# whwu95/MVFNet

Measured on AMD Instinct MI355X. Metric: clips/sec (fwd+bwd) MVFNet-R50 8x8 224^2, higher is better.
Workload: dtype bf16; 1 GPU; MVFNet-ResNet50 8x8, 32 clips/GPU of 8x3x224x224, bf16, train step: fwd (batch-stat BN) + loss + bwd + clip + SGD-nesterov; all through the HIP C ABI (stem + 16 bottlenecks + MVF + TSN head); clips_per_gpu=32, frames_per_clip=8, parallelism=dp1: replicas, one flat gradient all-reduce per step

## Files before the change

### mvfnet_amd/csrc/conv_nhwc.hip

```cpp
#include <algorithm>
#include <type_traits>
#include <stdlib.h>
#include <string.h>

#include "common.h"

namespace {

constexpr int kThreads = 256;
constexpr int kPitch = 144;
constexpr int kBM = 128;

typedef float f32x16 __attribute__((ext_vector_type(16)));
typedef short bf16x8 __attribute__((ext_vector_type(8)));

struct ConvArgs {
    const char* x;
    const char* x2;
    const char* w;
    const char* res;
    const float* bias;
    char* y;
    int N, H, W, Cin, Cout, KH, KW, stride, pad, Ho, Wo;
    int xps, split_c, x2ps, relu;
// ... 742 lines not shown
            }
        }
        if (wm == 0) __builtin_amdgcn_s_barrier();
        asm volatile("s_waitcnt vmcnt(0)" ::: "memory");
        __syncthreads();
#undef MVF_PIN2
    } else if constexpr (GLDS >= 2) {
        if (nseg > 0) load_chunk(s0, 0);
        for (int kc = 0; kc < nseg; ++kc) {
            asm volatile("s_waitcnt vmcnt(0)" ::: "memory");
            __syncthreads();
#ifdef MVF_CONV_ABLATE
            if (kc + 1 < nseg && !(a.prio & 4)) load_chunk(s0, (kc + 1) & 1);
            if (!(a.prio & 2)) compute(kc & 1);
#else
            if constexpr (ILV) {
                const bool more = kc + 1 < nseg;
                if (more) prep_chunk((kc + 1) & 1);
                compute(kc & 1, more);
            } else {
                if (kc + 1 < nseg) load_chunk(s0, (kc + 1) & 1);
                compute(kc & 1);
            }
#endif
        }
        __syncthreads();
    } else if constexpr (LOWK) {
        if (nseg > 0) {
            load_chunk(s0);
            store_chunk(0, s0);
        }
        __syncthreads();
        for (int kc = 0; kc < nseg; ++kc) {
            const bool more = kc + 1 < nseg;
            if (more) load_chunk(s0);
            compute(0);
            if (more) {
                __syncthreads();
                store_chunk(0, s0);
            }
            __syncthreads();
        }
    } else if constexpr (PF2) {
        load_chunk(s0);
        load_chunk(s1);
        if (nseg > 0) store_chunk(0, s0);
        __syncthreads();
        load_chunk(s0);
        int kc = 0;
        for (; kc + 1 < nseg; kc += 2) {
            compute(0);
            store_chunk(1, s1);
            load_chunk(s1);
            __syncthreads();
            compute(1);
            if (kc + 2 < nseg) store_chunk(0, s0);
            load_chunk(s0);
            __syncthreads();
        }
        if (kc < nseg) {
            compute(0);
            __syncthreads();
        }
    } else {
        if (nseg > 0) {
            load_chunk(s0);
            store_chunk(0, s0);
        }
        __syncthreads();
        for (int kc = 0; kc < nseg; ++kc) {
            const int buf = kc & 1;
            const bool more = kc + 1 < nseg;
            if (more) load_chunk(s0);
            compute(buf);
            if (more) store_chunk(buf ^ 1, s0);
            __syncthreads();
        }
    }

#ifdef MVF_CONV_ABLATE
    if (a.prio & 16) return;
#endif
    if (mode == SEG_PRODUCE) {
        float* slot = sk.ws + (long)g_self * (BM * BN);
#pragma unroll
        for (int i = 0; i < TM; ++i)
#pragma unroll
            for (int j = 0; j < TN; ++j)
#pragma unroll
                for (int r = 0; r < 16; ++r) slot[((i * TN + j) * 16 + r) * NT + tid] = acc[i][j][r];
        asm volatile("s_waitcnt vmcnt(0)" ::: "memory");
        __syncthreads();
        if (tid == 0) {
            __builtin_amdgcn_fence(__ATOMIC_RELEASE, "agent");
            asm volatile("s_waitcnt vmcnt(0)" ::: "memory");
            __hip_atomic_store(sk.flags + g_self, 1u, __ATOMIC_RELAXED, __HIP_MEMORY_SCOPE_AGENT);
        }
        return;
    }
    if (mode == SEG_FINISH) {
        for (int g = g_first; g < g_self; ++g) {
            if (tid == 0) {
                unsigned spins = 0;
                while (__hip_atomic_load(sk.flags + g, __ATOMIC_RELAXED, __HIP_MEMORY_SCOPE_AGENT) == 0u) {
                    __builtin_amdgcn_s_sleep(4);
                    if (++spins > (1u << 26)) {
                        __hip_atomic_store(sk.err, 1u, __ATOMIC_RELAXED, __HIP_MEMORY_SCOPE_AGENT);
                        break;
                    }
                }
                __builtin_amdgcn_fence(__ATOMIC_ACQUIRE, "agent");
            }
            __syncthreads();
            const float* slot = sk.ws + (long)g * (BM * BN);
#pragma unroll
            for (int i = 0; i < TM; ++i)
#pragma unroll
                for (int j = 0; j < TN; ++j)
#pragma unroll
                    for (int r = 0; r < 16; ++r) acc[i][j][r] += slot[((i * TN + j) * 16 + r) * NT + tid];
        }
    }

    const bool e_bias = EPI == 0 ? a.bias != nullptr : (EPI == 4 || EPI == 5 || (EPI == 6 && a.bias != nullptr));
    const bool e_res = EPI == 0 ? a.res != nullptr : (EPI == 3 || EPI == 5 || EPI == 8 || EPI == 9 || EPI == 10 || EPI == 12);
    constexpr bool e_bw = EPI == 9 || EPI == 10;
    const bool e_relu = EPI == 0 ? a.relu != 0 : (EPI == 4 || EPI == 5);
    constexpr bool e_apply = EPI == 8;
    const bool e_stats = EPI == 0 ? a.stats_part != nullptr : (EPI == 1 || EPI == 12);
    constexpr bool e_bnb = EPI == 6;
    const bool e_scatter = (EPI == 0 || EPI == 6) && a.o_s > 0;
    constexpr int CP = BN * 4 + 16;
    constexpr int NH = (LOWK || GLDS) ? 2 : 1;
    constexpr int HR = BM / NH;
    static_assert(HR * CP <= kSmem, "C tile (or half) must fit in the A/B LDS buffers");
    static_assert(HR % 32 == 0, "half split follows the MFMA row tiles");
    constexpr int PPT = BM / kBM;
    constexpr int HPP = NH / PPT;
    static_assert(NH % PPT == 0 && HPP >= 1, "a statistics partial covers whole epilogue passes");
    constexpr int TPR = BN / 4, RPP = NT / TPR;
    const int cq = tid % TPR, r0 = tid / TPR;
    const int col = n0 + cq * 4;
    ET* y = reinterpret_cast<ET*>(a.y);
    const ET* res = reinterpret_cast<const ET*>(a.res);
    float4 bv = make_float4(0.f, 0.f, 0.f, 0.f);
    if (e_bias && col < a.Cout) bv = *reinterpret_cast<const float4*>(a.bias + col);
    float4 st1 = make_float4(0.f, 0.f, 0.f, 0.f), st2 = st1, kk = st1;
    if (e_stats && a.stats_shift && col < a.Cout) kk = *reinterpret_cast<const float4*>(a.stats_shift + col);
    float4 ap_s = st1, ap_b = st1, ap_rs = make_float4(1.f, 1.f, 1.f, 1.f), ap_rb = st1;
    if (e_apply && col < a.Cout) {
        ap_s = *reinterpret_cast<const float4*>(a.ap_scale + col); ap_b = *reinterpret_cast<const float4*>(a.ap_shift + col);
        if (a.ap_rscale) { ap_rs = *reinterpret_cast<const float4*>(a.ap_rscale + col); ap_rb = *reinterpret_cast<const float4*>(a.ap_rshift + col); }
    }
    float4 b_mu = st1, b_rs = st1, b_sc = st1, b_sh = st1;
    if (e_bnb && col < a.Cout) {
        b_mu = *reinterpret_cast<const float4*>(a.bn_mean + col); b_rs = *reinterpret_cast<const float4*>(a.bn_invstd + col);
        b_sc = *reinterpret_cast<const float4*>(a.bn_scale + col); b_sh = *reinterpret_cast<const float4*>(a.bn_shift + col);
    }
    float4 w_a = st1, w_d0 = st1, w_kx = st1;
    if (e_bw && col < a.Cout) {
        b_mu = *reinterpret_cast<const float4*>(a.bn_mean + col); b_rs = *reinterpret_cast<const float4*>(a.bn_invstd + col);
        if constexpr (EPI == 9) {
            const float inv_m = 1.0f / (float)a.M;
            const float4 ga = *reinterpret_cast<const float4*>(a.bw_gamma + col), dg = *reinterpret_cast<const float4*>(a.bw_dgamma + col),
                         db = *reinterpret_cast<const float4*>(a.bw_dbeta + col);
            w_a = make_float4(ga.x * b_rs.x, ga.y * b_rs.y, ga.z * b_rs.z, ga.w * b_rs.w);
            w_d0 = make_float4(db.x * inv_m, db.y * inv_m, db.z * inv_m, db.w * inv_m);
            w_kx = make_float4(b_rs.x * dg.x * inv_m, b_rs.y * dg.y * inv_m, b_rs.z * dg.z * inv_m, b_rs.w * dg.w * inv_m);
        }
    }
    typedef unsigned u32x2 __attribute__((ext_vector_type(2)));
    const int eimg0 = fd_div(m0, a.fd_hw_mul, a.fd_hw_shr);
    __amdgpu_buffer_rsrc_t rs_y, rs_res;
    {
        const long total = (e_scatter ? (long)a.N * a.o_hfull * a.o_wfull : (long)a.M) * a.Cout * ESZ;
        const long base = (e_scatter ? (long)eimg0 * a.o_hfull * a.o_wfull : (long)m0) * a.Cout * ESZ;
        const long left = total - base;
        const unsigned nrec = (unsigned)(left < 0x7ffffff0L ? left : 0x7ffffff0L);
        rs_y = __builtin_amdgcn_make_buffer_rsrc((void*)(a.y + base), 0, a.y ? nrec : 0u, 0x00020000);
        rs_res = __builtin_amdgcn_make_buffer_rsrc((void*)(e_res ? a.res + base : (e_bnb ? a.bn_z + base : a.y + base)), 0, nrec, 0x00020000);
    }
    const __amdgpu_buffer_rsrc_t rs_mask = __builtin_amdgcn_make_buffer_rsrc(
        (void*)(a.res_mask ? a.res_mask + (long)m0 * (a.Cout / 4) : (const unsigned char*)a.y), 0,
        (unsigned)min((long)(a.M - m0) * (a.Cout / 4), 0x7ffffff0L), 0x00020000);
    const __amdgpu_buffer_rsrc_t rs_gate = __builtin_amdgcn_make_buffer_rsrc(
        (void*)(a.out_gate ? a.out_gate + (long)m0 * (a.Cout / 4) : (const unsigned char*)a.y), 0,
        (unsigned)min((long)(a.M - m0) * (a.Cout / 4), 0x7ffffff0L), 0x00020000);
    const bool e_gate = e_res && !e_apply && !e_bw && a.out_gate != nullptr;
    (void)y; (void)res;
    constexpr int kMaskOff = HR * CP;
    constexpr int MSEG = BN / 64;
    static_assert(kMaskOff + BM * (BN / 4) <= kSmem, "mask tile must fit behind the C tile");
    const bool mask_lds = e_res && (a.res_mask || e_gate) && (a.Cout % 64 == 0) && a.mask_lds;
    if (mask_lds) {
#pragma unroll
        for (int it = tid; it < BM * MSEG; it += NT) {
            const int row = it / MSEG, seg = it - row * MSEG;
            const unsigned moff = (unsigned)(row * (a.Cout / 4) + n0 / 4 + seg * 16);
            u32x4 mv = {0x0f0f0f0fu, 0x0f0f0f0fu, 0x0f0f0f0fu, 0x0f0f0f0fu};
            if (a.res_mask) mv = __builtin_amdgcn_raw_buffer_load_b128(rs_mask, moff, 0, 0);
            if (e_gate) {
                const u32x4 gv = __builtin_amdgcn_raw_buffer_load_b128(rs_gate, moff, 0, 0);
                mv.x = (mv.x & 0x0f0f0f0fu) | ((gv.x & 0x0f0f0f0fu) << 4); mv.y = (mv.y & 0x0f0f0f0fu) | ((gv.y & 0x0f0f0f0fu) << 4);
// ... 503 lines not shown
        default: return false;
    }
}

template <typename ET, int WM, int WN, int TM, int TN, int EPI>
void launch_lowk(bool pw, int tiles, size_t lds, hipStream_t st, const ConvArgs& a) {
    if constexpr (sizeof(ET) == 4) {
        if (x3_on(a)) {
            constexpr size_t lds3 = (size_t)kLowkLdsX3<WM * TM * 32, WN * TN * 32>();
            if constexpr (WN * TN * 32 == 128 && EPI >= 1 && EPI <= 6) {
                const int t_wide = ((a.M + 255) / 256) * a.tiles_n;
                if (g_x3_wide > 0 && t_wide >= g_x3_wide) {
                    ConvArgs b = a;
                    b.tiles_m = (a.M + 255) / 256;
                    constexpr size_t ldsw = (size_t)kLowkLdsX3<256, 128>();
                    auto k0 = conv_igemm_x3w_kernel<EPI, false>;
                    auto k1 = conv_igemm_x3w_kernel<EPI, true>;
                    static bool attrw = false;
                    if (!attrw) {
                        (void)hipFuncSetAttribute((const void*)k0, hipFuncAttributeMaxDynamicSharedMemorySize, (int)ldsw);
                        (void)hipFuncSetAttribute((const void*)k1, hipFuncAttributeMaxDynamicSharedMemorySize, (int)ldsw);
                        attrw = true;
                    }
                    if (pw) hipLaunchKernelGGL(k1, dim3(t_wide), dim3(512), ldsw, st, b);
                    else hipLaunchKernelGGL(k0, dim3(t_wide), dim3(512), ldsw, st, b);
                    return;
                }
            }
            if constexpr (EPI >= 1 && EPI <= 6) {
                if (a.nchunks >= g_x3_db_min) {
                    constexpr size_t ldsdb = (size_t)2 * (WM * TM * 32 + WN * TN * 32) * 192;
                    auto k0 = conv_igemm_x3db_kernel<WM, WN, TM, TN, EPI, false>;
                    auto k1 = conv_igemm_x3db_kernel<WM, WN, TM, TN, EPI, true>;
                    static bool attr = false;
                    if (!attr) {
                        (void)hipFuncSetAttribute((const void*)k0, hipFuncAttributeMaxDynamicSharedMemorySize, (int)ldsdb);
                        (void)hipFuncSetAttribute((const void*)k1, hipFuncAttributeMaxDynamicSharedMemorySize, (int)ldsdb);
                        attr = true;
                    }
                    if (pw) hipLaunchKernelGGL(k1, dim3(tiles), dim3(kThreads), ldsdb, st, a);
                    else hipLaunchKernelGGL(k0, dim3(tiles), dim3(kThreads), ldsdb, st, a);
                    return;
                }
            }
            if (pw) hipLaunchKernelGGL((conv_igemm_x3_kernel<WM, WN, TM, TN, EPI, true>), dim3(tiles), dim3(kThreads), lds3, st, a);
            else hipLaunchKernelGGL((conv_igemm_x3_kernel<WM, WN, TM, TN, EPI, false>), dim3(tiles), dim3(kThreads), lds3, st, a);
            return;
        }
    }
    if (pw) {
        auto k = conv_igemm_lowk_kernel<ET, WM, WN, TM, TN, EPI, true>;
        hipLaunchKernelGGL(k, dim3(tiles), dim3(kThreads), lds, st, a);
    } else {
        auto k = conv_igemm_lowk_kernel<ET, WM, WN, TM, TN, EPI, false>;
        hipLaunchKernelGGL(k, dim3(tiles), dim3(kThreads), lds, st, a);
    }
}

template <typename ET, int WM, int WN, int TM, int TN>
__global__ __launch_bounds__(kThreads) void conv_streamk_kernel(ConvArgs a, SkArgs sk) {
    extern __shared__ __attribute__((aligned(16))) char smem[];
    const int g = blockIdx.x, nc = a.nchunks;
    auto start_of = [&](int w) { return w < sk.units_rem ? w * (sk.units_base + 1) : sk.units_rem * (sk.units_base + 1) + (w - sk.units_rem) * sk.units_base; };
    auto wg_of = [&](int u) {
        const int bnd = sk.units_rem * (sk.units_base + 1);
        return u < bnd ? u / (sk.units_base + 1) : sk.units_rem + (u - bnd) / sk.units_base;
    };
    const int u0 = start_of(g), u1 = start_of(g + 1);
    const int t_first = u0 / nc, t_last = (u1 - 1) / nc;
    const int cb_first = u0 - t_first * nc, ce_last = u1 - t_last * nc;
    const bool last_partial = ce_last < nc;
    if (last_partial) {
        const int cb = t_last == t_first ? cb_first : 0;
        conv_tile<ET, WM, WN, TM, TN>(a, smem, sk.tile0 + t_last, cb, ce_last, SEG_PRODUCE, sk, 0, g);
    }
    const int t_hi = last_partial ? t_last - 1 : t_last;
    for (int t = t_first + 1; t <= t_hi; ++t) conv_tile<ET, WM, WN, TM, TN>(a, smem, sk.tile0 + t, 0, nc, SEG_FULL, sk, 0, g);
    if (t_first <= t_hi) {
        if (cb_first == 0) conv_tile<ET, WM, WN, TM, TN>(a, smem, sk.tile0 + t_first, 0, nc, SEG_FULL, sk, 0, g);
        else conv_tile<ET, WM, WN, TM, TN>(a, smem, sk.tile0 + t_first, cb_first, nc, SEG_FINISH, sk, wg_of(t_first * nc), g);
    }
}

template <typename ET>
__global__ void pack_weight_kernel(const float* w, int cout, int cin, int kh, int kw, int kwp, int cinp,
                                   const float* scale, ET* out) {
    const long total = (long)cout * kh * kwp * cinp;
    for (long i = (long)blockIdx.x * blockDim.x + threadIdx.x; i < total; i += (long)gridDim.x * blockDim.x) {
        long t = i;
        const int ci = (int)(t % cinp); t /= cinp;
        const int x = (int)(t % kwp); t /= kwp;
        const int yk = (int)(t % kh); t /= kh;
        const int co = (int)t;
        float v = 0.f;
        if (ci < cin && x < kw) {
            v = w[(((long)co * cin + ci) * kh + yk) * kw + x];
            if (scale) v *= scale[co];
        }
        stf(out + i, v);
    }
}

__global__ void bn_fold_kernel(const float* gamma, const float* beta, const float* mean, const float* var, float eps,
                               int c, float* scale, float* shift) {
    int i = blockIdx.x * blockDim.x + threadIdx.x;
    if (i >= c) return;
    const float s = gamma[i] / sqrtf(var[i] + eps);
    scale[i] = s;
    shift[i] = beta[i] - mean[i] * s;
}

static inline bool contiguous_ok(const ConvArgs& a) { return a.o_s <= 0; }
struct SkHost {
    void* ws;
    size_t ws_bytes;
};

int g_lowk_max_chunks = 1 << 30;
int g_pf2_mode = 1;
int g_glds1_f32_infer = 1;
int g_glds1_max = -1;
int g_big_min = 0;
int g_big2_min = 16;
int g_glds_min = -1, g_glds_nb = 2;

int sk_slots() {
    static int slots = 0;
    if (!slots) {
        g_lowk_max_chunks = mvf_policy_int("conv_lowk", g_lowk_max_chunks);
        g_pf2_mode = mvf_policy_int("conv_pf2", g_pf2_mode);
        g_glds1_f32_infer = mvf_policy_int("conv_glds1_f32", g_glds1_f32_infer);
        g_glds1_max = mvf_policy_int("conv_glds1", g_glds1_max);
        g_f32_x3 = mvf_policy_int("f32_x3", g_f32_x3);
        g_x3_wide = mvf_policy_int("x3_wide", g_x3_wide);
        g_x3_db_min = mvf_policy_int("x3_db", g_x3_db_min);
        g_big_min = mvf_policy_int("conv_big", g_big_min);
        g_big2_min = mvf_policy_int("conv_big2", g_big2_min);
        g_glds_min = mvf_policy_int("conv_glds", g_glds_min);
        g_glds_nb = mvf_policy_int("conv_glds_nb", g_glds_nb);
        int dev = 0, cus = 256;
        if (hipGetDevice(&dev) == hipSuccess) {
            hipDeviceProp_t p;
            if (hipGetDeviceProperties(&p, dev) == hipSuccess && p.multiProcessorCount > 0) cus = p.multiProcessorCount;
        }
        slots = 2 * cus;
    }
    return slots;
}

float sk_min_us() {
    static const float v = (float)mvf_policy_int("sk_min_us", 60);
    return v;
}

size_t sk_ws_bytes() { return (size_t)sk_slots() * (128 * 128 * sizeof(float)) + 4096; }

template <typename ET, int WM, int WN, int TM, int TN>
int launch_conv(const ConvArgs& a0, const SkHost& skh, hipStream_t st) {
    ConvArgs a = a0;
    constexpr int BM = WM * TM * 32, BN = WN * TN * 32;
    a.tiles_m = (a.M + BM - 1) / BM;
    a.tiles_n = (a.Cout + BN - 1) / BN;
    fd_make((unsigned)(a.Ho * a.Wo), a.fd_hw_mul, a.fd_hw_shr);
    fd_make((unsigned)a.Wo, a.fd_w_mul, a.fd_w_shr);
    const size_t lds = (size_t)2 * (BM + BN) * kPitch;
    auto kern = conv_igemm_kernel<ET, WM, WN, TM, TN>;
    auto kern_sk = conv_streamk_kernel<ET, WM, WN, TM, TN>;
    auto kern_pf = conv_igemm_pf2_kernel<ET, WM, WN, TM, TN>;
    static bool attr_done = false;
    if (!attr_done) {
        MVF_HIP_OK(hipFuncSetAttribute((const void*)kern, hipFuncAttributeMaxDynamicSharedMemorySize, (int)lds));
        MVF_HIP_OK(hipFuncSetAttribute((const void*)kern_pf, hipFuncAttributeMaxDynamicSharedMemorySize, (int)lds));
        MVF_HIP_OK(hipFuncSetAttribute((const void*)kern_sk, hipFuncAttributeMaxDynamicSharedMemorySize, (int)lds));
        attr_done = true;
    }
    const int tiles = a.tiles_m * a.tiles_n, slots = sk_slots();
    const long img_bytes = (long)a.H * a.W * std::max(a.xps, a.x2ps) * (long)sizeof(ET);
    const long span_imgs = std::min<long>(a.N, 128L / std::max(1, a.Ho * a.Wo) + 2);
    MVF_REQUIRE(a.o_s <= 0 || (long)a.o_hfull * a.o_wfull * a.Cout * (long)sizeof(ET) * span_imgs < 0x7ffffff0L, MVF_EUNSUPPORTED,
                "conv2d: output image too large for tile-relative 32-bit addressing");
    MVF_REQUIRE(!a.bn_z || !(a.dil > 1 || a.KH > 31 || a.KW > 31 || img_bytes * span_imgs >= 0x7ffffff0L), MVF_EUNSUPPORTED,
                "conv2d_dgrad_bnsums: shape needs the generic kernel, which has no BatchNorm-backward epilogue");
    MVF_REQUIRE(!a.bw_mode || !(a.dil > 1 || a.KH > 31 || a.KW > 31 || img_bytes * span_imgs >= 0x7ffffff0L || a.o_s > 0), MVF_EUNSUPPORTED,
                "conv2d_fwd_bnbwd: shape needs the generic kernel / a scattered output, which have no BatchNorm-backward-on-recompute epilogue");
    MVF_REQUIRE(!a.ap_scale || !(a.dil > 1 || a.KH > 31 || a.KW > 31 || img_bytes * span_imgs >= 0x7ffffff0L || a.o_s > 0), MVF_EUNSUPPORTED,
                "conv2d_fwd_bnapply: shape needs the generic kernel / a scattered output, which have no BatchNorm-apply epilogue");
    if (a.dil > 1 || a.KH > 31 || a.KW > 31 || img_bytes * span_imgs >= 0x7ffffff0L || (long)a.Cout * a.wK * (long)sizeof(ET) >= 0x7ffffff0L) {
        auto kern_gen = conv_igemm_gen_kernel<ET, WM, WN, TM, TN>;
        static bool gen_attr = false;
        if (!gen_attr) {
            MVF_HIP_OK(hipFuncSetAttribute((const void*)kern_gen, hipFuncAttributeMaxDynamicSharedMemorySize, (int)lds));
            gen_attr = true;
        }
        hipLaunchKernelGGL(kern_gen, dim3(tiles), dim3(kThreads), lds, st, a);
        MVF_LAUNCH_CHECK();
        return MVF_OK;
    }
    bool sk_wins = false;
    {
        const int full0 = tiles / slots * slots, tail0 = tiles - full0;
        const float wave_us0 = a.nchunks * (sizeof(ET) == 4 ? 3.9f : 1.0f);
        sk_wins = skh.ws && skh.ws_bytes >= sk_ws_bytes() && tail0 > 0 && (long)tail0 * a.nchunks >= slots &&
                  (1.0f - (float)tail0 / slots) * wave_us0 > sk_min_us();
    }
    if (a.mvf_coef) {
        MVF_REQUIRE(a.KH == 1 && a.KW == 1 && a.stride == 1 && a.pad == 0 && a.pad_w == 0 && a.split_c == 0 && a.o_s <= 0 && a.bias && a.relu &&
                        !a.res && !a.stats_part && !a.bn_z, MVF_EINVAL, "conv2d_mvf: needs a plain 1x1 stride-1 conv with bias + ReLU");
        MVF_REQUIRE(img_bytes * (span_imgs + 1) < 0x7ffffff0L, MVF_EUNSUPPORTED, "conv2d_mvf: image too large for tile-relative 32-bit addressing");
        fd_make((unsigned)a.mvf_T, a.fd_t_mul, a.fd_t_shr);
        static const int fk_env = mvf_policy_int("fuse_kernel", -1);
        const int fk = fk_env >= 0 ? fk_env : (a.nchunks <= 16 ? 1 : 2);
        if (fk == 0) {
            auto k = conv_igemm_lowk_kernel<ET, WM, WN, TM, TN, 4, true, true>;
            constexpr size_t lds_mvf = (size_t)kLowkLds<BM, BN>();
            hipLaunchKernelGGL(k, dim3(tiles), dim3(kThreads), lds_mvf, st, a);
        } else if (fk == 1) {
            auto k = conv_igemm_glds_kernel<ET, WM, WN, TM, TN, 4, 1, true>;
            constexpr size_t lds_mvf = (size_t)kGldsLds<BM, BN, 1>();
            hipLaunchKernelGGL(k, dim3(tiles), dim3(kThreads), lds_mvf, st, a);
        } else {
            auto k = conv_igemm_glds_kernel<ET, WM, WN, TM, TN, 4, 2, true>;
            constexpr size_t lds_mvf = (size_t)kGldsLds<BM, BN, 2>();
            static bool attr_mvf = false;
            if (!attr_mvf) {
                MVF_HIP_OK(hipFuncSetAttribute((const void*)k, hipFuncAttributeMaxDynamicSharedMemorySize, (int)lds_mvf));
                attr_mvf = true;
            }
            hipLaunchKernelGGL(k, dim3(tiles), dim3(kThreads), lds_mvf, st, a);
        }
        MVF_LAUNCH_CHECK();
        return MVF_OK;
    }
    if (a.bn_z || a.ap_scale || a.bw_mode) sk_wins = false;
    const bool x3 = sizeof(ET) == 4 && x3_on(a);
    if (x3) sk_wins = false;
    if ((a.nchunks <= g_lowk_max_chunks && !sk_wins) || a.bn_z || a.ap_scale || a.bw_mode || x3) {
        constexpr size_t lds_lk = (size_t)kLowkLds<BM, BN>();
        static const int epi_spec = mvf_policy_int("conv_epi", 3);
        const bool pw = (epi_spec & 2) && a.KH == 1 && a.KW == 1 && a.pad == 0 && a.pad_w == 0 && a.split_c == 0 && a.dil <= 1;
        const bool contiguous = (epi_spec & 1) && a.o_s <= 0;
        const bool train_like = contiguous && !a.bias && !a.relu;
        const bool infer_like = contiguous && a.bias && a.relu && !a.stats_part;
        const bool bnsum_epi = (epi_spec & 1) && a.bn_z && !a.relu && !a.res;
        if (BN == 128 && sizeof(ET) == 2 && g_big2_min > 0 && a.nchunks >= g_big2_min && a.Cout % 256 == 0 && a.o_s <= 0 && !a.ap_scale && !a.bw_mode) {
            const long t2 = (long)((a.M + 255) / 256) * (a.Cout / 256);
            const int cus = slots / 2;
            const long rounds = (t2 + cus - 1) / cus;
            static const bool force2 = mvf_policy_has("conv_big2_force");
            if (force2 || (t2 >= cus / 2 && (double)t2 / (double)(rounds * cus) >= 0.75)) {
                int rc;
                static const int p4_on = mvf_policy_int("conv_p4", 1);
                if (p4_on && a.Cin % 64 == 0 && (a.split_c % 64) == 0) {
                    if (train_like && a.stats_part && !a.res && !a.bn_z) rc = launch_p4<ET, 1>(st, a);
                    else if (bnsum_epi) rc = launch_p4<ET, 6>(st, a);
                    else if (train_like && !a.stats_part && !a.res) rc = launch_p4<ET, 2>(st, a);
                    else if (train_like && !a.stats_part && a.res) rc = launch_p4<ET, 3>(st, a);
                    else if (infer_like && !a.res) rc = launch_p4<ET, 4>(st, a);
                    else if (infer_like && a.res) rc = launch_p4<ET, 5>(st, a);
                    else rc = launch_p4<ET, 0>(st, a);
                    if (rc != MVF_OK) return rc;
                    MVF_LAUNCH_CHECK();
                    return MVF_OK;
                }
                if (train_like && a.stats_part && !a.res && !a.bn_z) rc = launch_big2<ET, 1>(st, a);
                else if (bnsum_epi) rc = launch_big2<ET, 6>(st, a);
                else if (train_like && !a.stats_part && !a.res) rc = launch_big2<ET, 2>(st, a);
                else if (train_like && !a.stats_part && a.res) rc = launch_big2<ET, 3>(st, a);
                else if (infer_like && !a.res) rc = launch_big2<ET, 4>(st, a);
                else if (infer_like && a.res) rc = launch_big2<ET, 5>(st, a);
                else rc = launch_big2<ET, 0>(st, a);
                if (rc != MVF_OK) return rc;
                MVF_LAUNCH_CHECK();
                return MVF_OK;
            }
        }
        if (BN == 128 && g_big_min > 0 && a.nchunks >= g_big_min && a.Cout >= 128 && a.M >= 256 && !a.ap_scale && !a.bw_mode) {
            int rc;
            if (train_like && a.stats_part && !a.res && !a.bn_z) rc = launch_big<ET, 1>(st, a);
            else if (bnsum_epi) rc = launch_big<ET, 6>(st, a);
            else if (train_like && !a.stats_part && !a.res) rc = launch_big<ET, 2>(st, a);
            else if (train_like && !a.stats_part && a.res) rc = launch_big<ET, 3>(st, a);
            else if (infer_like && !a.res) rc = launch_big<ET, 4>(st, a);
            else if (infer_like && a.res) rc = launch_big<ET, 5>(st, a);
            else rc = launch_big<ET, 0>(st, a);
            if (rc != MVF_OK) return rc;
            MVF_LAUNCH_CHECK();
            return MVF_OK;
        }
        const int glds1_max = x3 ? 0 : g_glds1_max >= 0 ? g_glds1_max
                              : (sizeof(ET) == 2 ? (infer_like ? 16 : 8) : ((infer_like && g_glds1_f32_infer) ? 8 : 0));
        if (glds1_max > 0 && a.nchunks <= glds1_max && !((bnsum_epi || a.bw_mode == 10) && g_glds1_max < 0)) {
            int rc;
            if (a.ap_scale) rc = launch_glds<ET, WM, WN, TM, TN, 8>(1, tiles, st, a);
            else if (a.bw_mode == 9) rc = launch_glds<ET, WM, WN, TM, TN, 9>(1, tiles, st, a);
            else if (a.bw_mode == 10) rc = launch_glds<ET, WM, WN, TM, TN, 10>(1, tiles, st, a);
            else if (train_like && a.stats_part && !a.res && !a.bn_z) rc = launch_glds<ET, WM, WN, TM, TN, 1>(1, tiles, st, a);
            else if (bnsum_epi) rc = launch_glds<ET, WM, WN, TM, TN, 6>(1, tiles, st, a);
            else if (train_like && !a.stats_part && !a.res) rc = launch_glds<ET, WM, WN, TM, TN, 2>(1, tiles, st, a);
            else if (train_like && !a.stats_part && a.res) rc = launch_glds<ET, WM, WN, TM, TN, 3>(1, tiles, st, a);
            else if (train_like && a.stats_part && a.res && a.out_gate && !a.bn_z) rc = launch_glds<ET, WM, WN, TM, TN, 12>(1, tiles, st, a);
            else if (infer_like && !a.res) rc = launch_glds<ET, WM, WN, TM, TN, 4>(1, tiles, st, a);
            else if (infer_like && a.res) rc = launch_glds<ET, WM, WN, TM, TN, 5>(1, tiles, st, a);
            else rc = launch_glds<ET, WM, WN, TM, TN, 0>(1, tiles, st, a);
            if (rc != MVF_OK) return rc;
            MVF_LAUNCH_CHECK();
            return MVF_OK;
        }
        const bool glds_auto = g_glds_min < 0 && sizeof(ET) == 2 && (a.nchunks >= 32 || (BN == 64 && a.nchunks >= 9));
        if (!x3 && ((g_glds_min > 0 && a.nchunks >= g_glds_min) || glds_auto)) {
            int rc;
            if (a.ap_scale) rc = launch_glds<ET, WM, WN, TM, TN, 8>(g_glds_nb, tiles, st, a);
            else if (a.bw_mode == 9) rc = launch_glds<ET, WM, WN, TM, TN, 9>(g_glds_nb, tiles, st, a);
            else if (a.bw_mode == 10) rc = launch_glds<ET, WM, WN, TM, TN, 10>(g_glds_nb, tiles, st, a);
            else if (train_like && a.stats_part && !a.res && !a.bn_z) rc = launch_glds<ET, WM, WN, TM, TN, 1>(g_glds_nb, tiles, st, a);
            else if (bnsum_epi) rc = launch_glds<ET, WM, WN, TM, TN, 6>(g_glds_nb, tiles, st, a);
            else if (train_like && !a.stats_part && !a.res) rc = launch_glds<ET, WM, WN, TM, TN, 2>(g_glds_nb, tiles, st, a);
            else if (train_like && !a.stats_part && a.res) rc = launch_glds<ET, WM, WN, TM, TN, 3>(g_glds_nb, tiles, st, a);
            else if (train_like && a.stats_part && a.res && a.out_gate && !a.bn_z) rc = launch_glds<ET, WM, WN, TM, TN, 12>(g_glds_nb, tiles, st, a);
            else if (infer_like && !a.res) rc = launch_glds<ET, WM, WN, TM, TN, 4>(g_glds_nb, tiles, st, a);
            else if (infer_like && a.res) rc = launch_glds<ET, WM, WN, TM, TN, 5>(g_glds_nb, tiles, st, a);
            else rc = launch_glds<ET, WM, WN, TM, TN, 0>(g_glds_nb, tiles, st, a);
            if (rc != MVF_OK) return rc;
            MVF_LAUNCH_CHECK();
            return MVF_OK;
        }
        if (a.ap_scale) launch_lowk<ET, WM, WN, TM, TN, 8>(pw, tiles, lds_lk, st, a);
        else if (a.bw_mode == 9) launch_lowk<ET, WM, WN, TM, TN, 9>(pw, tiles, lds_lk, st, a);
        else if (a.bw_mode == 10) launch_lowk<ET, WM, WN, TM, TN, 10>(pw, tiles, lds_lk, st, a);
        else if (train_like && a.stats_part && !a.res && !a.bn_z) launch_lowk<ET, WM, WN, TM, TN, 1>(pw, tiles, lds_lk, st, a);
        else if (bnsum_epi) launch_lowk<ET, WM, WN, TM, TN, 6>(pw, tiles, lds_lk, st, a);
        else if (train_like && !a.stats_part && !a.res) launch_lowk<ET, WM, WN, TM, TN, 2>(pw, tiles, lds_lk, st, a);
        else if (train_like && !a.stats_part && a.res) launch_lowk<ET, WM, WN, TM, TN, 3>(pw, tiles, lds_lk, st, a);
        else if (train_like && a.stats_part && a.res && a.out_gate && !a.bn_z) launch_lowk<ET, WM, WN, TM, TN, 12>(pw, tiles, lds_lk, st, a);
        else if (infer_like && !a.res) launch_lowk<ET, WM, WN, TM, TN, 4>(pw, tiles, lds_lk, st, a);
        else if (infer_like && a.res) launch_lowk<ET, WM, WN, TM, TN, 5>(pw, tiles, lds_lk, st, a);
        else launch_lowk<ET, WM, WN, TM, TN, 0>(pw, tiles, lds_lk, st, a);
        MVF_LAUNCH_CHECK();
        return MVF_OK;
    }
    const int full = tiles / slots * slots, tail = tiles - full;
    const float wave_us = a.nchunks * (sizeof(ET) == 4 ? 3.9f : 1.0f);
    const bool use_sk = skh.ws && skh.ws_bytes >= sk_ws_bytes() && tail > 0 && (long)tail * a.nchunks >= slots &&
                        (1.0f - (float)tail / slots) * wave_us > sk_min_us();
    if (!use_sk) {
        const bool pf2 = g_pf2_mode == 2 || (g_pf2_mode == 1 && sizeof(ET) == 2);
        hipLaunchKernelGGL(pf2 ? kern_pf : kern, dim3(tiles), dim3(kThreads), lds, st, a);
        MVF_LAUNCH_CHECK();
        return MVF_OK;
    }
    if (full > 0) {
        hipLaunchKernelGGL(kern, dim3(full), dim3(kThreads), lds, st, a);
        MVF_LAUNCH_CHECK();
    }
    SkArgs sk;
    const long units = (long)tail * a.nchunks;
    sk.G = slots;
    sk.units_base = (int)(units / sk.G);
    sk.units_rem = (int)(units % sk.G);
    sk.tile0 = full;
    sk.ws = (float*)skh.ws;
    sk.flags = (unsigned*)((char*)skh.ws + (size_t)slots * (128 * 128 * sizeof(float)));
    sk.err = sk.flags + slots;
    MVF_HIP_OK(hipMemsetAsync(sk.flags, 0, (size_t)(slots + 1) * sizeof(unsigned), st));
    hipLaunchKernelGGL(kern_sk, dim3(sk.G), dim3(kThreads), lds, st, a, sk);
    MVF_LAUNCH_CHECK();
    return MVF_OK;
}

}

extern "C" {

size_t mvf_conv2d_workspace_bytes(const mvf_conv_desc_t*) { return sk_ws_bytes(); }

int mvf_conv2d_nhwc_fwd(const mvf_conv_desc_t* d, const void* x, const void* x2, const void* w_packed,
                        const float* bias, const void* residual, void* y, void* stream) {
    return mvf_conv2d_nhwc_fwd_ws(d, x, x2, w_packed, bias, residual, y, nullptr, 0, stream);
}

struct BnBwdSums {
    const void* z;
    const float *mean, *invstd, *scale, *shift;
};
struct MvfFuse {
    const float* coef;
    int cs, T, act;
};
struct BnBwdRecompute {
    int mode;
    const float *mean, *invstd, *gamma, *dgamma, *dbeta;
};
struct BnApply {
    const float *scale, *shift, *rscale, *rshift;
    unsigned char* bits;
};
static int conv_fwd_impl(const mvf_conv_desc_t* d, const void* x, const void* x2, const void* w_packed, const float* bias,
                         const void* residual, void* y, float* stats_part, const float* stats_shift, void* ws, size_t ws_bytes,
                         void* stream, const unsigned char* res_mask = nullptr, const BnBwdSums* bnb = nullptr, const MvfFuse* mf = nullptr,
                         const BnApply* ap = nullptr, const BnBwdRecompute* bw = nullptr, const unsigned char* out_gate = nullptr);

int mvf_conv2d_nhwc_fwd_mvf(const mvf_conv_desc_t* d, const void* x, const void* w_packed, const float* bias, const float* mvf_coef,
                            int cs, int n_segment, int act, void* y, void* ws, size_t ws_bytes, void* stream) {
    MVF_REQUIRE(d && mvf_coef && bias && cs > 0 && n_segment > 0, MVF_EINVAL, "conv2d_fwd_mvf: bad argument");
    const int ce = d->dtype == MVF_F32 ? 32 : 64;
    MVF_REQUIRE(cs % ce == 0 && cs <= d->cin && d->n % n_segment == 0 && d->ho == d->h && d->wo == d->w && d->x_pix_stride == d->cin, MVF_ESHAPE,
                "conv2d_fwd_mvf: cs=%d must be a multiple of %d (one K chunk), n a multiple of n_segment, output size = input size", cs, ce);
    MVF_REQUIRE((uintptr_t)mvf_coef % 16 == 0, MVF_EINVAL, "conv2d_fwd_mvf: mvf_coef must be 16-byte aligned");
    const MvfFuse mf = {mvf_coef, cs, n_segment, act};
    return conv_fwd_impl(d, x, nullptr, w_packed, bias, nullptr, y, nullptr, nullptr, ws, ws_bytes, stream, nullptr, nullptr, &mf);
}

int mvf_conv2d_nhwc_dgrad_bnsums(const mvf_conv_desc_t* d, const void* dz, const void* w_packed_dgrad, void* y, const void* bn_z,
                                 const float* bn_mean, const float* bn_invstd, const float* bn_scale, const float* bn_shift,
                                 float* sums_part, void* ws, size_t ws_bytes, void* stream) {
    MVF_REQUIRE(d && bn_z && bn_mean && bn_invstd && bn_scale && bn_shift && sums_part, MVF_EINVAL, "conv2d_dgrad_bnsums: NULL argument");
    const BnBwdSums b = {bn_z, bn_mean, bn_invstd, bn_scale, bn_shift};
    return conv_fwd_impl(d, dz, nullptr, w_packed_dgrad, nullptr, nullptr, y, sums_part, nullptr, ws, ws_bytes, stream, nullptr, &b);
}

int mvf_conv2d_nhwc_fwd_bnapply(const mvf_conv_desc_t* d, const void* x, const void* x2, const void* w_packed, const float* bn_scale,
                                const float* bn_shift, const void* residual, const float* res_scale, const float* res_shift, void* out,
                                unsigned char* sign_bits, void* ws, size_t ws_bytes, void* stream) {
    MVF_REQUIRE(d && bn_scale && bn_shift && residual && sign_bits, MVF_EINVAL, "conv2d_fwd_bnapply: NULL argument");
    MVF_REQUIRE((res_scale == nullptr) == (res_shift == nullptr), MVF_EINVAL, "conv2d_fwd_bnapply: res_scale / res_shift must come together");
    MVF_REQUIRE(d->in_dil <= 1 && !d->relu && d->cout % 4 == 0, MVF_EINVAL, "conv2d_fwd_bnapply: a forward launch (in_dil <= 1), relu = 0 in the descriptor");
    MVF_REQUIRE(((uintptr_t)bn_scale | (uintptr_t)bn_shift | (uintptr_t)(res_scale ? res_scale : bn_scale) | (uintptr_t)(res_shift ? res_shift : bn_shift)) % 16 == 0,
                MVF_EINVAL, "conv2d_fwd_bnapply: coefficient vectors must be 16-byte aligned");
    const BnApply ap = {bn_scale, bn_shift, res_scale, res_shift, sign_bits};
    return conv_fwd_impl(d, x, x2, w_packed, nullptr, residual, out, nullptr, nullptr, ws, ws_bytes, stream, nullptr, nullptr, nullptr, &ap);
}

int mvf_conv2d_nhwc_fwd_bnbwd_sums(const mvf_conv_desc_t* d, const void* x, const void* x2, const void* w_packed, const void* g,
                                   const unsigned char* sign_bits, const float* bn_mean, const float* bn_invstd, float* sums_part, void* ws,
                                   size_t ws_bytes, void* stream) {
    MVF_REQUIRE(d && g && sign_bits && bn_mean && bn_invstd && sums_part, MVF_EINVAL, "conv2d_fwd_bnbwd_sums: NULL argument");
    MVF_REQUIRE(d->in_dil <= 1 && !d->relu, MVF_EINVAL, "conv2d_fwd_bnbwd_sums: a forward launch (in_dil <= 1), relu = 0");
    MVF_REQUIRE(((uintptr_t)bn_mean | (uintptr_t)bn_invstd) % 16 == 0, MVF_EINVAL, "conv2d_fwd_bnbwd_sums: coefficient vectors must be 16-byte aligned");
    const BnBwdRecompute bw = {10, bn_mean, bn_invstd, nullptr, nullptr, nullptr};
    return conv_fwd_impl(d, x, x2, w_packed, nullptr, g, nullptr, sums_part, nullptr, ws, ws_bytes, stream, sign_bits, nullptr, nullptr, nullptr, &bw);
}

int mvf_conv2d_nhwc_fwd_bnbwd_apply(const mvf_conv_desc_t* d, const void* x, const void* x2, const void* w_packed, const void* g,
                                    const unsigned char* sign_bits, const float* bn_gamma, const float* bn_mean, const float* bn_invstd,
                                    const float* dgamma, const float* dbeta, void* dz, void* ws, size_t ws_bytes, void* stream) {
// ... 236 lines not shown
```

Baseline: 1775 clips/s.

## Add stream-K split-K conv kernel for training stats/bnsum epilogues

```diff
diff --git a/mvfnet_amd/csrc/conv_nhwc.hip b/mvfnet_amd/csrc/conv_nhwc.hip
--- a/mvfnet_amd/csrc/conv_nhwc.hip
+++ b/mvfnet_amd/csrc/conv_nhwc.hip
@@ -848,13 +848,14 @@
     if (a.prio & 16) return;
 #endif
     if (mode == SEG_PRODUCE) {
-        float* slot = sk.ws + (long)g_self * (BM * BN);
+        float4* slot = reinterpret_cast<float4*>(sk.ws + (long)g_self * (BM * BN));
 #pragma unroll
         for (int i = 0; i < TM; ++i)
 #pragma unroll
             for (int j = 0; j < TN; ++j)
 #pragma unroll
-                for (int r = 0; r < 16; ++r) slot[((i * TN + j) * 16 + r) * NT + tid] = acc[i][j][r];
+                for (int r = 0; r < 4; ++r)
+                    slot[((i * TN + j) * 4 + r) * NT + tid] = make_float4(acc[i][j][4 * r], acc[i][j][4 * r + 1], acc[i][j][4 * r + 2], acc[i][j][4 * r + 3]);
         asm volatile("s_waitcnt vmcnt(0)" ::: "memory");
         __syncthreads();
         if (tid == 0) {
@@ -878,13 +879,21 @@
                 __builtin_amdgcn_fence(__ATOMIC_ACQUIRE, "agent");
             }
             __syncthreads();
-            const float* slot = sk.ws + (long)g * (BM * BN);
+            const float4* slot = reinterpret_cast<const float4*>(sk.ws + (long)g * (BM * BN));
 #pragma unroll
             for (int i = 0; i < TM; ++i)
 #pragma unroll
                 for (int j = 0; j < TN; ++j)
-#pragma unroll
-                    for (int r = 0; r < 16; ++r) acc[i][j][r] += slot[((i * TN + j) * 16 + r) * NT + tid];
+                {
+                    float4 v[4];
+#pragma unroll
+                    for (int r = 0; r < 4; ++r) v[r] = slot[((i * TN + j) * 4 + r) * NT + tid];
+#pragma unroll
+                    for (int r = 0; r < 4; ++r) {
+                        acc[i][j][4 * r] += v[r].x; acc[i][j][4 * r + 1] += v[r].y; acc[i][j][4 * r + 2] += v[r].z; acc[i][j][4 * r + 3] += v[r].w;
+                    }
+                    __builtin_amdgcn_sched_barrier(0);
+                }
         }
     }
 
@@ -1554,6 +1563,50 @@
     }
 }
 
+struct SktArgs {
+    float* ws;
+    unsigned* flags;
+    unsigned* err;
+    int G, nx, tiles;
+};
+template <typename ET, int WM, int WN, int TM, int TN, int EPI, int GL>
+__global__ __launch_bounds__(WM * WN * 64, WM * WN == 4 ? 2 : 1) void conv_ksplit_kernel(ConvArgs a, SktArgs s) {
+    extern __shared__ __attribute__((aligned(16))) char smem[];
+    const int nx = s.nx, x = blockIdx.x % nx, idx = blockIdx.x / nx, nc = a.nchunks;
+    auto part0 = [](int n, int parts, int i) { const int q = n / parts, r = n % parts; return i < r ? i * (q + 1) : r * (q + 1) + (i - r) * q; };
+    const int t0 = part0(s.tiles, nx, x), tcnt = part0(s.tiles, nx, x + 1) - t0;
+    const int w0 = part0(s.G, nx, x), W = part0(s.G, nx, x + 1) - w0;
+    const int U = tcnt * nc, ub = U / W, ur = U % W;
+    auto start_of = [&](int w) { return w < ur ? w * (ub + 1) : ur * (ub + 1) + (w - ur) * ub; };
+    auto wg_of = [&](int u) { const int bnd = ur * (ub + 1); return u < bnd ? u / (ub + 1) : ur + (u - bnd) / ub; };
+    const int u0 = start_of(idx), u1 = start_of(idx + 1);
+    if (u0 >= u1) return;
+    const int t_first = u0 / nc, t_last = (u1 - 1) / nc;
+    const int cb_first = u0 - t_first * nc, ce_last = u1 - t_last * nc;
+    const bool last_partial = ce_last < nc;
+    const int t_hi = last_partial ? t_last - 1 : t_last;
+    const int n_whole = t_hi > t_first ? t_hi - t_first : 0;
+    const int nseg = (last_partial ? 1 : 0) + n_whole + (t_first <= t_hi ? 1 : 0);
+    SkArgs sk = {};
+    sk.ws = s.ws; sk.flags = s.flags; sk.err = s.err;
+    for (int sg = 0; sg < nseg; ++sg) {
+        int tile, cb = 0, ce = nc, mode = SEG_FULL, gf = 0, k = sg;
+        if (last_partial && k == 0) {
+            tile = t_last; cb = t_last == t_first ? cb_first : 0; ce = ce_last; mode = SEG_PRODUCE;
+        } else {
+            if (last_partial) --k;
+            if (k < n_whole) tile = t_first + 1 + k;
+            else {
+                tile = t_first; cb = cb_first;
+                if (cb_first != 0) { mode = SEG_FINISH; gf = w0 + wg_of(t_first * nc); }
+            }
+        }
+        conv_tile<ET, WM, WN, TM, TN, false, false, false, EPI, false, GL>(a, smem, __builtin_amdgcn_readfirstlane(t0 + tile), __builtin_amdgcn_readfirstlane(cb),
+                                                                           __builtin_amdgcn_readfirstlane(ce), __builtin_amdgcn_readfirstlane(mode), sk,
+                                                                           __builtin_amdgcn_readfirstlane(gf), w0 + idx);
+    }
+}
+
 template <typename ET>
 __global__ void pack_weight_kernel(const float* w, int cout, int cin, int kh, int kw, int kwp, int cinp,
                                    const float* scale, ET* out) {
@@ -1625,7 +1678,50 @@
     return v;
 }
 
-size_t sk_ws_bytes() { return (size_t)sk_slots() * (128 * 128 * sizeof(float)) + 4096; }
+size_t sk_ws_bytes() { return (size_t)(sk_slots() / 2) * (256 * 256 * sizeof(float)) + 4096; }
+
+constexpr float KS_US_CHUNK_128 = 1.0f, KS_US_CHUNK_256 = 1.8f;
+constexpr int KS_PRICE_US_128 = 29;
+int ksplit_mode() {
+    static const int mode = mvf_policy_int("conv_sk_train", 1);
+    return mode;
+}
+template <int BM>
+int ksplit_wgs(const ConvArgs& a, int tiles, const SkHost& skh) {
+    const int mode = ksplit_mode();
+    if (mode <= 0 || !skh.ws || skh.ws_bytes < sk_ws_bytes() || a.nchunks < 2 || tiles < 1) return 0;
+    const int cap = BM == 256 ? sk_slots() / 2 : sk_slots();
+    if (mode >= 2) {
+        const int g = mvf_policy_int("conv_sk_train_wgs", cap);
+        return g < 1 ? 1 : (g > cap ? cap : g);
+    }
+    static const float price = (float)mvf_policy_int("conv_sk_price", KS_PRICE_US_128);
+    const int rounds = (tiles + cap - 1) / cap;
+    const float split_rounds = (float)((tiles + 7) / 8) / (float)(cap / 8);
+    const float saving = ((float)rounds - split_rounds) * a.nchunks * (BM == 256 ? KS_US_CHUNK_256 : KS_US_CHUNK_128);
+    return saving > (BM == 256 ? 4.f * price : price) ? cap : 0;
+}
+template <typename ET, int WM, int WN, int TM, int TN, int EPI, int GL>
+int launch_ksplit(int G, int tiles, hipStream_t st, const ConvArgs& a, const SkHost& skh) {
+    constexpr int BM = WM * TM * 32, BN = WN * TN * 32, NT = WM * WN * 64;
+    constexpr int lds = kGldsLds<BM, BN, 2>();
+    auto k = conv_ksplit_kernel<ET, WM, WN, TM, TN, EPI, GL>;
+    static bool attr = false;
+    if (!attr) {
+        MVF_HIP_OK(hipFuncSetAttribute((const void*)k, hipFuncAttributeMaxDynamicSharedMemorySize, lds));
+        attr = true;
+    }
+    SktArgs s;
+    s.ws = (float*)skh.ws;
+    s.flags = (unsigned*)((char*)skh.ws + sk_ws_bytes() - 4096);
+    s.err = s.flags + sk_slots();
+    s.G = G;
+    s.nx = (G >= 64 && G % 8 == 0) ? 8 : 1;
+    s.tiles = tiles;
+    MVF_HIP_OK(hipMemsetAsync(s.flags, 0, (size_t)(sk_slots() + 1) * sizeof(unsigned), st));
+    hipLaunchKernelGGL(k, dim3(G), dim3(NT), lds, st, a, s);
+    return MVF_OK;
+}
 
 template <typename ET, int WM, int WN, int TM, int TN>
 int launch_conv(const ConvArgs& a0, const SkHost& skh, hipStream_t st) {
@@ -1723,6 +1819,19 @@
                 int rc;
                 static const int p4_on = mvf_policy_int("conv_p4", 1);
                 if (p4_on && a.Cin % 64 == 0 && (a.split_c % 64) == 0) {
+                    if constexpr (sizeof(ET) == 2) {
+                        const int ks_epi = (train_like && a.stats_part && !a.res && !a.bn_z) ? 1 : (bnsum_epi ? 6 : 0);
+                        const int G = (ks_epi && a.KH * a.KW > 1) ? ksplit_wgs<256>(a, (int)t2, skh) : 0;
+                        if (G > 0) {
+                            ConvArgs b = a;
+                            b.tiles_m = (a.M + 255) / 256;
+                            b.tiles_n = a.Cout / 256;
+                            rc = ks_epi == 1 ? launch_ksplit<ET, 2, 4, 4, 2, 1, 4>(G, (int)t2, st, b, skh) : launch_ksplit<ET, 2, 4, 4, 2, 6, 4>(G, (int)t2, st, b, skh);
+                            if (rc != MVF_OK) return rc;
+                            MVF_LAUNCH_CHECK();
+                            return MVF_OK;
+                        }
+                    }
                     if (train_like && a.stats_part && !a.res && !a.bn_z) rc = launch_p4<ET, 1>(st, a);
                     else if (bnsum_epi) rc = launch_p4<ET, 6>(st, a);
                     else if (train_like && !a.stats_part && !a.res) rc = launch_p4<ET, 2>(st, a);
@@ -1758,6 +1867,17 @@
             if (rc != MVF_OK) return rc;
             MVF_LAUNCH_CHECK();
             return MVF_OK;
+        }
+        if constexpr (sizeof(ET) == 2 && BM == 128 && BN == 128) {
+            const int ks_epi = (train_like && a.stats_part && !a.res && !a.bn_z) ? 1 : (bnsum_epi ? 6 : 0);
+            const bool ks_route = ksplit_mode() >= 2 || (g_glds_min < 0 && g_glds1_max < 0 && g_glds_nb == 2 && a.nchunks >= 32);
+            const int G = (ks_epi && ks_route && a.KH * a.KW > 1) ? ksplit_wgs<128>(a, tiles, skh) : 0;
+            if (G > 0) {
+                const int rc = ks_epi == 1 ? launch_ksplit<ET, WM, WN, TM, TN, 1, 2>(G, tiles, st, a, skh) : launch_ksplit<ET, WM, WN, TM, TN, 6, 2>(G, tiles, st, a, skh);
+                if (rc != MVF_OK) return rc;
+                MVF_LAUNCH_CHECK();
+                return MVF_OK;
+            }
         }
         const int glds1_max = x3 ? 0 : g_glds1_max >= 0 ? g_glds1_max
                               : (sizeof(ET) == 2 ? (infer_like ? 16 : 8) : ((infer_like && g_glds1_f32_infer) ? 8 : 0));
@@ -1831,7 +1951,7 @@
     sk.units_rem = (int)(units % sk.G);
     sk.tile0 = full;
     sk.ws = (float*)skh.ws;
-    sk.flags = (unsigned*)((char*)skh.ws + (size_t)slots * (128 * 128 * sizeof(float)));
+    sk.flags = (unsigned*)((char*)skh.ws + sk_ws_bytes() - 4096);
     sk.err = sk.flags + slots;
     MVF_HIP_OK(hipMemsetAsync(sk.flags, 0, (size_t)(slots + 1) * sizeof(unsigned), st));
     hipLaunchKernelGGL(kern_sk, dim3(sk.G), dim3(kThreads), lds, st, a, sk);
```

After: 1777 clips/s (median of 3 runs). Within noise of the previous version (+0.1%).
